# genomicepidemiology/ccphylo

Measured on AMD Instinct MI355X. Metric: taxa-pairs/sec (dist) + NJ iterations/sec at N taxa, 1/2/4/8 MI355X, higher is better.
Workload: dtype u2 packed codes -> MX-fp4 MFMA (exact integer counts), f64 LT and tree

## Files before the change

### ccphylo_amd/csrc/snp.hip

```cpp
#include <cstring>
#include <vector>
#include <type_traits>
#include "ccg_internal.h"
#include "ccg_shard_layout.h"

#define TILE 128
#define KC 16
#define KCP 8
#define RS 130
#define RSP 130

__device__ __forceinline__ uint32_t xor_or(uint32_t a, uint32_t b, uint32_t c) {
	return __builtin_amdgcn_bitop3_b32(a, b, c, 0xBE);
}

__device__ __forceinline__ uint32_t compress_even(uint64_t x) {
	x &= 0x5555555555555555ull;
	x = (x | (x >> 1)) & 0x3333333333333333ull;
	x = (x | (x >> 2)) & 0x0F0F0F0F0F0F0F0Full;
	x = (x | (x >> 4)) & 0x00FF00FF00FF00FFull;
	x = (x | (x >> 8)) & 0x0000FFFF0000FFFFull;
	x = (x | (x >> 16)) & 0x00000000FFFFFFFFull;
	return (uint32_t) x;
}
// ... 408 lines not shown
	int lo = 0, hi = npanels - 1;
	while(lo < hi) {
		const int mid = (lo + hi + 1) >> 1;
		if(pfx[mid] <= t) lo = mid; else hi = mid - 1;
	}
	const int I = lo, J = (int) (t - pfx[lo]);
	const Shard sh{rank, world};
	const auto arow = [&](int l) -> long long {
		const long long L = (long long) I * TILE + l, lb = L / SB, g = lb * world + rank, r = g * SB + (L - lb * SB);
		return r < n ? r : 0;
	};
	const uint2 *Bp = P + (size_t) J * TILE * Wp + wb;
	const int Wl = SPLIT ? (wb + Wk < Wp ? Wk : Wp - wb) : Wp;
	const int lane = threadIdx.x & 63, wid = threadIdx.x >> 6;
	const int wr = wid >> 1, wc = wid & 1;
	v16f_t acc[2][2];
#pragma unroll
	for(int a = 0; a < 2; ++a)
#pragma unroll
		for(int c = 0; c < 2; ++c)
#pragma unroll
			for(int r = 0; r < 16; ++r) acc[a][c][r] = 0.0f;
	uint4 va[4], vb[4];
	long long ar[4];
#pragma unroll
	for(int q = 0; q < 4; ++q) {
		const int e = q * 256 + threadIdx.x, row = e >> 3, wp = e & 7;
		ar[q] = arow(row);
		va[q] = *(const uint4 *) (P + (size_t) ar[q] * Wp + wb + 2 * wp);
		vb[q] = *(const uint4 *) (Bp + (size_t) row * Wp + 2 * wp);
	}
#pragma unroll
	for(int q = 0; q < 4; ++q) {
		const int e = q * 256 + threadIdx.x, row = e >> 3, wp = e & 7;
		As[0][(2 * wp) * RS + row] = make_uint2(va[q].x, va[q].y);
		As[0][(2 * wp + 1) * RS + row] = make_uint2(va[q].z, va[q].w);
		Bs[0][(2 * wp) * RS + row] = make_uint2(vb[q].x, vb[q].y);
		Bs[0][(2 * wp + 1) * RS + row] = make_uint2(vb[q].z, vb[q].w);
	}
	__syncthreads();
	const int h = lane >> 5, l32 = lane & 31;
	const int ra0 = 64 * wr + l32, rb0 = 64 * wc + l32;
	int buf = 0;
	for(int w0 = 0; w0 < Wl; w0 += KC, buf ^= 1) {
		const bool more = w0 + KC < Wl;
		if(more) {
#pragma unroll
			for(int q = 0; q < 4; ++q) {
				const int e = q * 256 + threadIdx.x, row = e >> 3, wp = e & 7;
				va[q] = *(const uint4 *) (P + (size_t) ar[q] * Wp + wb + w0 + KC + 2 * wp);
				vb[q] = *(const uint4 *) (Bp + (size_t) row * Wp + w0 + KC + 2 * wp);
			}
		}
		const uint2 *Ac = As[buf], *Bc = Bs[buf];
#pragma unroll 2
		for(int s = 0; s < KC / 2; ++s) {
			const int w = 2 * s + h;
			uint2 a[2], b[2];
#pragma unroll
			for(int tt = 0; tt < 2; ++tt) {
				a[tt] = Ac[w * RS + ra0 + 32 * tt];
				b[tt] = Bc[w * RS + rb0 + 32 * tt];
			}
#pragma unroll
			for(int comp = 0; comp < 3; ++comp) {
				v8i_t fa[2], fb[2];
#pragma unroll
				for(int tt = 0; tt < 2; ++tt) {
					fa[tt] = fp4_spread(comp == 0 ? a[tt].x : comp == 1 ? a[tt].y : a[tt].x ^ a[tt].y);
					fb[tt] = fp4_spread(comp == 0 ? b[tt].x : comp == 1 ? b[tt].y : b[tt].x ^ b[tt].y);
				}
#pragma unroll
				for(int ta = 0; ta < 2; ++ta)
#pragma unroll
					for(int tb = 0; tb < 2; ++tb)
						acc[ta][tb] = __builtin_amdgcn_mfma_scale_f32_32x32x64_f8f6f4(
						    fa[ta], fb[tb], acc[ta][tb], MFMA_FP4, MFMA_FP4, 0, MFMA_SCALE1, 0, MFMA_SCALE1);
			}
		}
		if(more) {
			uint2 *An = As[buf ^ 1], *Bn = Bs[buf ^ 1];
#pragma unroll
			for(int q = 0; q < 4; ++q) {
				const int e = q * 256 + threadIdx.x, row = e >> 3, wp = e & 7;
				An[(2 * wp) * RS + row] = make_uint2(va[q].x, va[q].y);
				An[(2 * wp + 1) * RS + row] = make_uint2(va[q].z, va[q].w);
				Bn[(2 * wp) * RS + row] = make_uint2(vb[q].x, vb[q].y);
				Bn[(2 * wp + 1) * RS + row] = make_uint2(vb[q].z, vb[q].w);
			}
		}
		__syncthreads();
	}
	const int L3 = 3 * 32 * Wl;
#pragma unroll
	for(int ta = 0; ta < 2; ++ta) {
#pragma unroll
		for(int r = 0; r < 16; ++r) {
			const int l = 64 * wr + 32 * ta + (r & 3) + 8 * (r >> 2) + 4 * h;
			const long long L = (long long) I * TILE + l, lb = L / SB, i = (lb * world + rank) * SB + (L - lb * SB);
			if(i >= n) continue;
			const long long base = sh.off(i);
#pragma unroll
			for(int tb = 0; tb < 2; ++tb) {
				const long long j = (long long) J * TILE + 64 * wc + 32 * tb + l32;
				if(j < i) {
					const unsigned d = (unsigned) ((L3 - (int) acc[ta][tb][r]) >> 2);
					if(SPLIT) atomicAdd(&cnt[base + j], d);
					else Dloc[base + j] = Elem<ET>::put(nFactor * (double) d, 0.5, bs);
				}
			}
		}
	}
}

#define TILE2 256
#define KC2 8
#define KC2L 16
#define RS2 260

__device__ __forceinline__ void tile_ij_super(long long t, long long Ihi, int &I, int &J) {
	int r, c;
	tile_ij(t, r, c);
	const long long P = r >> 2, I0 = 4 * P;
	if(I0 + 3 > Ihi) {
		I = r;
		J = c;
		return;
	}
	const long long u = t - I0 * (I0 + 1) / 2, F = P >> 1;
	if(u < 32 * F) {
		const int v = (int) (u & 31);
		I = (int) I0 + (v >> 3);
		J = 8 * (int) (u >> 5) + (v & 7);
		return;
	}
	long long w = u - 32 * F;
	int i = (int) I0;
	while(w >= i - 8 * F + 1) {
		w -= i - 8 * F + 1;
		++i;
	}
	I = i;
	J = (int) (8 * F + w);
}

__device__ __forceinline__ v8i_t fp4_xor_spread(const v8i_t &a, const v8i_t &b) {
	v8i_t v;
#pragma unroll
	for(int q = 0; q < 4; ++q) v[q] = (int) xor_or((uint32_t) a[q], (uint32_t) b[q], 0x22222222u);
	v[4] = v[5] = v[6] = v[7] = 0;
	return v;
}

template <int ET, bool SPLIT, bool BAND, int KCW = KC2>
__global__ __launch_bounds__(256, 1) void k_snp_mfma2(const uint2 *__restrict__ P, int Wp, int n, long long t0,
                                                      long long items, int S, int Wk, double nFactor, double bs,
                                                      typename Elem<ET>::T *__restrict__ D, long long rowBegin,
                                                      long long rowEnd, unsigned *__restrict__ cnt, long long cbase,
                                                      const long long *__restrict__ pfx, int npanels, int rank,
                                                      int world, int sorder) {
	constexpr int QS2 = TILE2 * KCW / 2 / 256, WPR = KCW / 2;
	__shared__ __attribute__((aligned(16))) uint2 As[2][KCW * RS2];
	__shared__ __attribute__((aligned(16))) uint2 Bs[2][KCW * RS2];
	const long long item = t0 + xcd_tile(blockIdx.x, items), t = SPLIT ? item / S : item;
	int I, J;
	if(BAND) {
		int lo = 0, hi = npanels - 1;
		while(lo < hi) {
			const int mid = (lo + hi + 1) >> 1;
			if(pfx[mid] <= t) lo = mid; else hi = mid - 1;
		}
		I = lo;
		J = (int) (t - pfx[lo]);
	} else if(sorder) {
		tile_ij_super(t, (rowEnd - 1) / TILE2, I, J);
	} else {
		tile_ij(t, I, J);
	}
	const int wb = SPLIT ? (int) (item % S) * Wk : 0;
	const int Wl = SPLIT ? (wb + Wk < Wp ? Wk : Wp - wb) : Wp;
	const Shard sh{rank, world};
	const auto arow = [&](int l) -> long long {
		const long long L = (long long) I * TILE2 + l;
		if(!BAND) return L;
		const long long lb = L / SB, r = (lb * world + rank) * SB + (L - lb * SB);
		return r < n ? r : 0;
	};
	const uint2 *Bp = P + (size_t) J * TILE2 * Wp + wb;
	long long ar[QS2];
	uint4 va[QS2], vb[QS2];
#pragma unroll
	for(int q = 0; q < QS2; ++q) {
		const int e = q * 256 + threadIdx.x, row = e / WPR, wp = e % WPR;
		ar[q] = arow(row);
		va[q] = *(const uint4 *) (P + (size_t) ar[q] * Wp + wb + 2 * wp);
		vb[q] = *(const uint4 *) (Bp + (size_t) row * Wp + 2 * wp);
	}
#pragma unroll
	for(int q = 0; q < QS2; ++q) {
		const int e = q * 256 + threadIdx.x, row = e / WPR, wp = e % WPR;
		As[0][(2 * wp) * RS2 + row] = make_uint2(va[q].x, va[q].y);
		As[0][(2 * wp + 1) * RS2 + row] = make_uint2(va[q].z, va[q].w);
		Bs[0][(2 * wp) * RS2 + row] = make_uint2(vb[q].x, vb[q].y);
		Bs[0][(2 * wp + 1) * RS2 + row] = make_uint2(vb[q].z, vb[q].w);
	}
	__syncthreads();
	const int lane = threadIdx.x & 63, wid = threadIdx.x >> 6;
	const int wr = wid >> 1, wc = wid & 1;
	const int h = lane >> 5, l32 = lane & 31;
	const int ra0 = 128 * wr + l32, rb0 = 128 * wc + l32;
	v16f_t acc[4][4];
#pragma unroll
	for(int a = 0; a < 4; ++a)
#pragma unroll
		for(int c = 0; c < 4; ++c)
#pragma unroll
			for(int r = 0; r < 16; ++r) acc[a][c][r] = 0.0f;
	int buf = 0;
	for(int w0 = 0; w0 < Wl; w0 += KCW, buf ^= 1) {
		const bool more = w0 + KCW < Wl;
		if(more) {
#pragma unroll
			for(int q = 0; q < QS2; ++q) {
				const int e = q * 256 + threadIdx.x, row = e / WPR, wp = e % WPR;
				va[q] = *(const uint4 *) (P + (size_t) ar[q] * Wp + wb + w0 + KCW + 2 * wp);
				vb[q] = *(const uint4 *) (Bp + (size_t) row * Wp + w0 + KCW + 2 * wp);
			}
		}
		const uint2 *Ac = As[buf], *Bc = Bs[buf];
#pragma unroll
		for(int s = 0; s < KCW / 2; ++s) {
			const int w = 2 * s + h;
			uint2 a[4], b[4];
#pragma unroll
			for(int x = 0; x < 4; ++x) {
				a[x] = Ac[w * RS2 + ra0 + 32 * x];
				b[x] = Bc[w * RS2 + rb0 + 32 * x];
			}
			v8i_t f0[4], g0[4], f1[4], g1[4];
#pragma unroll
			for(int x = 0; x < 4; ++x) {
				f0[x] = fp4_spread(a[x].x);
				g0[x] = fp4_spread(b[x].x);
			}
#pragma unroll
			for(int ta = 0; ta < 4; ++ta)
#pragma unroll
				for(int tb = 0; tb < 4; ++tb)
					acc[ta][tb] = __builtin_amdgcn_mfma_scale_f32_32x32x64_f8f6f4(
					    f0[ta], g0[tb], acc[ta][tb], MFMA_FP4, MFMA_FP4, 0, MFMA_SCALE1, 0, MFMA_SCALE1);
#pragma unroll
			for(int x = 0; x < 4; ++x) {
				f1[x] = fp4_spread(a[x].y);
				g1[x] = fp4_spread(b[x].y);
			}
#pragma unroll
			for(int ta = 0; ta < 4; ++ta)
#pragma unroll
				for(int tb = 0; tb < 4; ++tb)
					acc[ta][tb] = __builtin_amdgcn_mfma_scale_f32_32x32x64_f8f6f4(
					    f1[ta], g1[tb], acc[ta][tb], MFMA_FP4, MFMA_FP4, 0, MFMA_SCALE1, 0, MFMA_SCALE1);
#pragma unroll
			for(int x = 0; x < 4; ++x) {
				f0[x] = fp4_xor_spread(f0[x], f1[x]);
				g0[x] = fp4_xor_spread(g0[x], g1[x]);
			}
#pragma unroll
			for(int ta = 0; ta < 4; ++ta)
#pragma unroll
				for(int tb = 0; tb < 4; ++tb)
					acc[ta][tb] = __builtin_amdgcn_mfma_scale_f32_32x32x64_f8f6f4(
					    f0[ta], g0[tb], acc[ta][tb], MFMA_FP4, MFMA_FP4, 0, MFMA_SCALE1, 0, MFMA_SCALE1);
		}
		if(more) {
			uint2 *An = As[buf ^ 1], *Bn = Bs[buf ^ 1];
#pragma unroll
			for(int q = 0; q < QS2; ++q) {
				const int e = q * 256 + threadIdx.x, row = e / WPR, wp = e % WPR;
				An[(2 * wp) * RS2 + row] = make_uint2(va[q].x, va[q].y);
				An[(2 * wp + 1) * RS2 + row] = make_uint2(va[q].z, va[q].w);
				Bn[(2 * wp) * RS2 + row] = make_uint2(vb[q].x, vb[q].y);
				Bn[(2 * wp + 1) * RS2 + row] = make_uint2(vb[q].z, vb[q].w);
			}
		}
		__syncthreads();
	}
	const int L3 = 3 * 32 * Wl;
#pragma unroll
	for(int ta = 0; ta < 4; ++ta) {
#pragma unroll
		for(int r = 0; r < 16; ++r) {
			const int l = 128 * wr + 32 * ta + (r & 3) + 8 * (r >> 2) + 4 * h;
			const long long L = (long long) I * TILE2 + l;
			long long i = L;
			if(BAND) {
				const long long lb = L / SB;
				i = (lb * world + rank) * SB + (L - lb * SB);
			}
			if(i >= n || (!BAND && (i < rowBegin || i >= rowEnd))) continue;
			const long long base = BAND ? sh.off(i) : tri(i);
#pragma unroll
			for(int tb = 0; tb < 4; ++tb) {
				const long long j = (long long) J * TILE2 + 128 * wc + 32 * tb + l32;
				if(j < i) {
					const unsigned d = (unsigned) ((L3 - (int) acc[ta][tb][r]) >> 2);
					if(SPLIT) {
						atomicAdd(&cnt[base + j - cbase], d);
					} else {
						const double v = nFactor * (double) d;
						D[base + j] = Elem<ET>::put(v, 0.5, bs);
					}
				}
			}
		}
	}
}

#define NST3 4
#define KC3 8
template <int ET, bool SPLIT, bool BAND>
__global__ __launch_bounds__(256, 1) void k_snp_mfma3(const uint2 *__restrict__ P, int Wp, int n, long long t0,
                                                      long long items, int S, int Wk, double nFactor, double bs,
                                                      typename Elem<ET>::T *__restrict__ D, long long rowBegin,
                                                      long long rowEnd, unsigned *__restrict__ cnt, long long cbase,
                                                      const long long *__restrict__ pfx, int npanels, int rank,
                                                      int world, int sorder) {
	constexpr int NSL = KC3 / 2;
	static_assert(NSL == 4, "one slice per wave");
	__shared__ __attribute__((aligned(16))) uint4 L[NST3 * 2 * NSL * TILE2];
	const long long item = t0 + xcd_tile(blockIdx.x, items), t = SPLIT ? item / S : item;
	int I, J;
	if(BAND) {
		int lo = 0, hi = npanels - 1;
		while(lo < hi) {
			const int mid = (lo + hi + 1) >> 1;
			if(pfx[mid] <= t) lo = mid; else hi = mid - 1;
		}
		I = lo;
		J = (int) (t - pfx[lo]);
	} else if(sorder) {
		tile_ij_super(t, (rowEnd - 1) / TILE2, I, J);
	} else {
		tile_ij(t, I, J);
	}
	const int wb = SPLIT ? (int) (item % S) * Wk : 0;
	const int Wl = SPLIT ? (wb + Wk < Wp ? Wk : Wp - wb) : Wp;
	const Shard sh{rank, world};
	const int lane = threadIdx.x & 63, wid = threadIdx.x >> 6;
	const uint2 *srcA[4], *srcB[4];
#pragma unroll
	for(int q = 0; q < 4; ++q) {
		const long long Lr = (long long) I * TILE2 + q * 64 + lane;
		long long r = Lr;
		if(BAND) {
			const long long lb = Lr / SB;
			r = (lb * world + rank) * SB + (Lr - lb * SB);
			r = r < n ? r : 0;
		}
		srcA[q] = P + (size_t) r * Wp + wb + 2 * wid;
		srcB[q] = P + ((size_t) J * TILE2 + q * 64 + lane) * Wp + wb + 2 * wid;
	}
	const int nch = Wl / KC3;
	const unsigned lbase = (unsigned) (uintptr_t) (__attribute__((address_space(3))) uint4 *) L;
	auto glds = [&](const uint2 *src, unsigned lds) {
		unsigned keep;
		asm volatile("s_mov_b32 %0, m0\n\ts_mov_b32 m0, %2\n\ts_nop 0\n\tglobal_load_lds_dwordx4 %1, off\n\ts_mov_b32 m0, %0"
		             : "=&s"(keep)
		             : "v"(src), "s"(lds)
		             : "memory");
	};
	auto issue = [&](int c) {
		const int st = c % NST3, w0 = c * KC3;
#pragma unroll
		for(int q = 0; q < 4; ++q) {
			glds(srcA[q] + w0, __builtin_amdgcn_readfirstlane(lbase + (unsigned) ((((st * 2 + 0) * NSL + wid) * TILE2 + q * 64) * 16)));
			glds(srcB[q] + w0, __builtin_amdgcn_readfirstlane(lbase + (unsigned) ((((st * 2 + 1) * NSL + wid) * TILE2 + q * 64) * 16)));
		}
	};
	const int wr = wid >> 1, wc = wid & 1;
	const int h = lane >> 5, l32 = lane & 31;
	const int ra0 = 128 * wr + l32, rb0 = 128 * wc + l32;
	v16f_t acc[4][4];
#pragma unroll
	for(int ta = 0; ta < 4; ++ta)
#pragma unroll
		for(int tb = 0; tb < 4; ++tb)
#pragma unroll
			for(int r = 0; r < 16; ++r) acc[ta][tb][r] = 0.0f;
	auto land = [&](int c) {
		const int ahead = nch - 1 - c < NST3 - 2 ? nch - 1 - c : NST3 - 2;
		if(ahead >= 2) asm volatile("s_waitcnt vmcnt(16)" ::: "memory");
		else if(ahead == 1) asm volatile("s_waitcnt vmcnt(8)" ::: "memory");
		else asm volatile("s_waitcnt vmcnt(0)" ::: "memory");
		asm volatile("" ::: "memory");
		__builtin_amdgcn_s_barrier();
		asm volatile("" ::: "memory");
	};
	auto rd = [&](int gs, uint2 (&a)[4], uint2 (&b)[4]) {
		const int st = (gs >> 2) % NST3, sl = gs & 3;
		const uint2 *Ac = (const uint2 *) &L[((st * 2 + 0) * NSL + sl) * TILE2];
		const uint2 *Bc = (const uint2 *) &L[((st * 2 + 1) * NSL + sl) * TILE2];
#pragma unroll
		for(int x = 0; x < 4; ++x) {
			a[x] = Ac[(ra0 + 32 * x) * 2 + h];
			b[x] = Bc[(rb0 + 32 * x) * 2 + h];
		}
	};
#define MF3(TA, TB, F, G)                                                                                         \
	acc[TA][TB] = __builtin_amdgcn_mfma_scale_f32_32x32x64_f8f6f4(F, G, acc[TA][TB], MFMA_FP4, MFMA_FP4, 0, MFMA_SCALE1, \
	                                                              0, MFMA_SCALE1)
	for(int c = 0; c < NST3 - 1 && c < nch; ++c) issue(c);
	land(0);
	if(NST3 - 1 < nch) issue(NST3 - 1);
	uint2 a[4], b[4];
	v8i_t f0[4], g0[4];
	rd(0, a, b);
#pragma unroll
	for(int x = 0; x < 4; ++x) {
		f0[x] = fp4_spread(a[x].x);
		g0[x] = fp4_spread(b[x].x);
	}
	auto step = [&](auto SI, int gs, bool more, bool open) {
		constexpr int G0 = 3 * decltype(SI)::value;
		v8i_t f1[4], g1[4], x0[4], y0[4];
#pragma unroll
		for(int k = 0; k < 16; ++k) {
			MF3(k >> 2, k & 3, f0[k >> 2], g0[k & 3]);
			if(k < 8) {
				if(k & 1) g1[k >> 1] = fp4_spread(b[k >> 1].y);
				else f1[k >> 1] = fp4_spread(a[k >> 1].y);
			}
		}
#pragma unroll
		for(int k = 0; k < 8; ++k) {
			__builtin_amdgcn_sched_group_barrier(0x008, 1, G0);
			__builtin_amdgcn_sched_group_barrier(0x002, 7, G0);
		}
		__builtin_amdgcn_sched_group_barrier(0x008, 8, G0);
		if(open) {
			const int cn = (gs + 1) >> 2;
			land(cn);
			if(cn + NST3 - 1 < nch) issue(cn + NST3 - 1);
		}
		uint2 an[4], bn[4];
		if(more) rd(gs + 1, an, bn);
#pragma unroll
		for(int k = 0; k < 16; ++k) {
			MF3(k >> 2, k & 3, f1[k >> 2], g1[k & 3]);
			if(k < 8) {
				if(k & 1) y0[k >> 1] = fp4_xor_spread(g0[k >> 1], g1[k >> 1]);
				else x0[k >> 1] = fp4_xor_spread(f0[k >> 1], f1[k >> 1]);
			}
		}
		if(more) __builtin_amdgcn_sched_group_barrier(0x100, 8, G0 + 1);
#pragma unroll
		for(int k = 0; k < 8; ++k) {
			__builtin_amdgcn_sched_group_barrier(0x008, 1, G0 + 1);
			__builtin_amdgcn_sched_group_barrier(0x002, 4, G0 + 1);
		}
		__builtin_amdgcn_sched_group_barrier(0x008, 8, G0 + 1);
#pragma unroll
		for(int k = 0; k < 16; ++k) {
			MF3(k >> 2, k & 3, x0[k >> 2], y0[k & 3]);
			if(more && k < 8) {
				if(k & 1) g0[k >> 1] = fp4_spread(bn[k >> 1].x);
				else f0[k >> 1] = fp4_spread(an[k >> 1].x);
			}
		}
		if(more) {
#pragma unroll
			for(int k = 0; k < 8; ++k) {
				__builtin_amdgcn_sched_group_barrier(0x008, 1, G0 + 2);
				__builtin_amdgcn_sched_group_barrier(0x002, 7, G0 + 2);
			}
			__builtin_amdgcn_sched_group_barrier(0x008, 8, G0 + 2);
#pragma unroll
			for(int x = 0; x < 4; ++x) {
				a[x] = an[x];
				b[x] = bn[x];
			}
		}
	};
	for(int c = 0; c + 1 < nch; ++c) {
		step(std::integral_constant<int, 0>(), 4 * c + 0, true, false);
		step(std::integral_constant<int, 1>(), 4 * c + 1, true, false);
		step(std::integral_constant<int, 2>(), 4 * c + 2, true, false);
		step(std::integral_constant<int, 3>(), 4 * c + 3, true, true);
	}
	{
		const int g = 4 * (nch - 1);
		step(std::integral_constant<int, 0>(), g + 0, true, false);
		step(std::integral_constant<int, 1>(), g + 1, true, false);
		step(std::integral_constant<int, 2>(), g + 2, true, false);
		step(std::integral_constant<int, 3>(), g + 3, false, false);
	}
#undef MF3
	const int L3 = 3 * 32 * Wl;
#pragma unroll
	for(int ta = 0; ta < 4; ++ta) {
#pragma unroll
		for(int r = 0; r < 16; ++r) {
			const int l = 128 * wr + 32 * ta + (r & 3) + 8 * (r >> 2) + 4 * h;
			const long long Lr = (long long) I * TILE2 + l;
			long long i = Lr;
			if(BAND) {
				const long long lb = Lr / SB;
				i = (lb * world + rank) * SB + (Lr - lb * SB);
			}
			if(i >= n || (!BAND && (i < rowBegin || i >= rowEnd))) continue;
			const long long base = BAND ? sh.off(i) : tri(i);
#pragma unroll
			for(int tb = 0; tb < 4; ++tb) {
				const long long j = (long long) J * TILE2 + 128 * wc + 32 * tb + l32;
				if(j < i) {
					const unsigned d = (unsigned) ((L3 - (int) acc[ta][tb][r]) >> 2);
					if(SPLIT) {
						atomicAdd(&cnt[base + j - cbase], d);
					} else {
						const double v = nFactor * (double) d;
						D[base + j] = Elem<ET>::put(v, 0.5, bs);
					}
				}
			}
		}
	}
}

template <int ET>
__global__ void k_snp_finish(const unsigned *__restrict__ cnt, long long cbase, long long f0, long long f1,
                             double nFactor, double bs, typename Elem<ET>::T *__restrict__ D) {
	for(long long f = f0 + (long long) blockIdx.x * blockDim.x + threadIdx.x; f < f1;
	    f += (long long) gridDim.x * blockDim.x) {
		D[f] = Elem<ET>::put(nFactor * (double) cnt[f - cbase], 0.5, bs);
	}
}

template <int ET>
__device__ __forceinline__ void pair_store(typename Elem<ET>::T *D, typename Elem<ET>::T *N, long long f, uint32_t dist,
                                           uint32_t inc, unsigned norm, unsigned minLength, double bs) {
	typedef typename Elem<ET>::T T;
	if(ET == 8) {
		double v;
		if(minLength <= inc) {
			v = norm ? (double) ((unsigned long long) dist * norm) / inc : (double) dist;
		} else {
			v = -1.0;
		}
		D[f] = (T) v;
		if(N) N[f] = (T) (double) inc;
	} else if(ET == 4) {
		float v;
		if(minLength <= inc) {
			if(norm) {
				v = (float) ((unsigned long long) dist * norm);
				v = v / (float) inc;
			} else {
				v = (float) dist;
			}
		} else {
			v = -1.0f;
		}
		D[f] = (T) v;
		if(N) N[f] = (T) (float) inc;
	} else {
		double v;
		if(minLength <= inc) {
			v = norm ? ((double) ((unsigned long long) dist * norm) * bs + 0.5) / inc : (double) dist * bs + 0.5;
		} else {
			v = -1.0 * bs + 0;
		}
		D[f] = (T) cvt_i32_x86(v);
		if(N) N[f] = (T) cvt_i32_x86(inc * bs + 0.5);
	}
}

template <int ET, bool SPLIT, bool BAND = false>
__global__ __launch_bounds__(256, 2) void k_snp_tile_pair(const uint4 *__restrict__ P, int Wp, int n, long long t0,
                                                          long long items, int S, int Wk, unsigned norm,
                                                          unsigned minLength, double bs,
                                                          typename Elem<ET>::T *__restrict__ D,
                                                          typename Elem<ET>::T *__restrict__ Nm, long long rowBegin,
                                                          long long rowEnd, unsigned *__restrict__ cd,
                                                          unsigned *__restrict__ cn, long long cbase,
                                                          const long long *__restrict__ pfx = nullptr, int npanels = 0,
                                                          int rank = 0, int world = 1) {
	__shared__ __attribute__((aligned(16))) uint4 As[2][KCP * RSP];
	__shared__ __attribute__((aligned(16))) uint4 Bs[2][KCP * RSP];
	int I, J;
	const long long item = t0 + xcd_tile(blockIdx.x, items);
	if(BAND) {
		const long long tile = item / S;
		int lo = 0, hi = npanels - 1;
		while(lo < hi) {
			const int mid = (lo + hi + 1) >> 1;
			if(pfx[mid] <= tile) lo = mid; else hi = mid - 1;
		}
		I = lo;
		J = (int) (tile - pfx[lo]);
	} else {
		tile_ij(item / S, I, J);
	}
	const auto arow = [&](int l) -> long long {
		const long long L = (long long) I * TILE + l;
		if(!BAND) return L;
		const long long lb = L / SB, r = (lb * world + rank) * SB + (L - lb * SB);
		return r < n ? r : 0;
	};
	const int wb = (int) (item % S) * Wk, we = wb + Wk < Wp ? wb + Wk : Wp;
	const int Wl = we - wb;
	const int tx = threadIdx.x & 15, ty = threadIdx.x >> 4;
	const uint4 *Aq[4];
#pragma unroll
	for(int q = 0; q < 4; ++q) Aq[q] = P + (size_t) arow((q * 256 + threadIdx.x) >> 3) * Wp + wb;
	const uint4 *Bp = P + (size_t) J * TILE * Wp + wb;
	uint32_t ad[8][8], an[8][8];
#pragma unroll
	for(int a = 0; a < 8; ++a)
#pragma unroll
		for(int c = 0; c < 8; ++c) {
			ad[a][c] = 0;
			an[a][c] = 0;
		}
	uint4 va[4], vb[4];
#pragma unroll
	for(int q = 0; q < 4; ++q) {
		const int e = q * 256 + threadIdx.x, row = e >> 3, wp = e & 7;
		va[q] = Aq[q][wp];
		vb[q] = Bp[(size_t) row * Wp + wp];
	}
#pragma unroll
	for(int q = 0; q < 4; ++q) {
		const int e = q * 256 + threadIdx.x, row = e >> 3, wp = e & 7;
		As[0][wp * RSP + row] = va[q];
		Bs[0][wp * RSP + row] = vb[q];
	}
	__syncthreads();
	int buf = 0;
	for(int w0 = 0; w0 < Wl; w0 += KCP, buf ^= 1) {
		const bool more = w0 + KCP < Wl;
		if(more) {
#pragma unroll
			for(int q = 0; q < 4; ++q) {
				const int e = q * 256 + threadIdx.x, row = e >> 3, wp = e & 7;
				va[q] = Aq[q][w0 + KCP + wp];
				vb[q] = Bp[(size_t) row * Wp + w0 + KCP + wp];
			}
		}
		const uint4 *Ac = As[buf], *Bc = Bs[buf];
#pragma unroll 1
// ... 489 lines not shown
			uint32_t m = 0, d = 0;
			if(w < W32) {
				const uint4 a = A[w], b = B[w];
				m = a.z & b.z;
				d = xor_or(a.x, b.x, a.y ^ b.y) & m;
			}
			cnt += __popc(m);
			dist += __popc(d);
			const int hiL = d ? 32 * w + 32 - (__ffs(d)) + 1 : -1;
			int incl = wave_scan_max_incl(hiL, lane);
			int prevL = __shfl_up(incl, 1, 64);
			if(lane == 0) prevL = -1;
			if(cL > prevL) prevL = cL;
			int qhi = 0;
			{
				int prev = prevL;
				for(uint32_t x = d; x;) {
					const int k = __clz(x);
					x &= ~(0x80000000u >> k);
					const int cur = 32 * w + k + 1;
					qhi = prev >= 0 && cur - prev <= proxi;
					prev = cur;
				}
			}
			const int packed = hiL >= 0 ? 2 * hiL + qhi : -1;
			const int incl2 = wave_scan_max_incl(packed, lane);
			int prevP = __shfl_up(incl2, 1, 64);
			if(lane == 0) prevP = -1;
			const int cP = cL >= 0 ? 2 * cL + cQ : -1;
			if(cP > prevP) prevP = cP;
			{
				int prev = prevL, qprev = prevP >= 0 ? (prevP & 1) : 0;
				for(uint32_t x = d; x;) {
					const int k = __clz(x);
					x &= ~(0x80000000u >> k);
					const int cur = 32 * w + k + 1;
					const int qc = prev >= 0 && cur - prev <= proxi;
					if(qc) {
						uint32_t rm, rd;
						range_counts(A, B, W32, prev, cur, rm, rd);
						cnt -= rm;
						dist -= rd;
						if(qprev) {
							range_counts(A, B, W32, prev, prev, rm, rd);
							cnt += rm;
							dist += rd;
						}
					}
					prev = cur;
					qprev = qc;
				}
			}
			const int top = __shfl(incl2, 63, 64);
			if(top >= 0 && (top >> 1) > cL) {
				cL = top >> 1;
				cQ = top & 1;
			}
		}
		if(lane == 0 && cL >= 0 && (long long) len + proxi - cL <= proxi) {
			uint32_t rm, rd;
			const long long e = (long long) len + proxi;
			range_counts(A, B, W32, cL, e < 32LL * W32 ? (int) e : 32 * W32 - 1, rm, rd);
			cnt -= rm;
			dist -= rd;
			if(cQ) {
				range_counts(A, B, W32, cL, cL, rm, rd);
				cnt += rm;
				dist += rd;
			}
		}
#pragma unroll
		for(int o = 32; o > 0; o >>= 1) {
			dist += __shfl_xor(dist, o, 64);
			cnt += __shfl_xor(cnt, o, 64);
		}
		if(lane == 0) pair_store<ET>(D, Nm, f, (uint32_t) dist, (uint32_t) cnt, norm, minLength, bs);
	}
}

static inline long long cdivll(long long a, long long b) { return (a + b - 1) / b; }

static int dist_kernel_choice() {
	const char *mf = getenv("CCG_DIST_MFMA");
	return mf ? atoi(mf) : 2;
}

template <int ET, bool PAIR = false>
static int snp_launch_mfma2(ccg_ctx *ctx, const ccg_snp_args *a, const void *planes, int Wp, double nFactor, void *D,
                            long long rb, long long re, int rank, int world, void *N = NULL) {
	typedef typename Elem<ET>::T T;
	const long long n = a->n;
	long long t_begin = 0, t_end = 0, f0 = 0, f1 = 0;
	int npanels = 0;
	long long *d_pfx = NULL;
	if(world > 0) {
		const long long nb = (n + SB - 1) / SB;
		long long nloc = 0;
		if(rank < nb) {
			const long long owned = (nb - 1 - rank) / world + 1, last = (owned - 1) * world + rank;
			nloc = (owned - 1) * SB + (n - last * SB < SB ? n - last * SB : SB);
		}
		npanels = (int) cdivll(nloc, TILE2);
		if(npanels == 0) return CCG_OK;
		std::vector<long long> pfx(npanels + 1, 0);
		for(long long I = 0; I < npanels; ++I) {
			const long long Lmax = (I + 1) * TILE2 - 1 < nloc - 1 ? (I + 1) * TILE2 - 1 : nloc - 1;
			const long long lb = Lmax / SB, rmax = (lb * world + rank) * SB + (Lmax - lb * SB);
			pfx[I + 1] = pfx[I] + cdivll(rmax, TILE2);
		}
		CCG_CHECK(hipMalloc(&d_pfx, (size_t) (npanels + 1) * sizeof(long long)));
		if(hipMemcpyAsync(d_pfx, pfx.data(), (size_t) (npanels + 1) * sizeof(long long), hipMemcpyHostToDevice,
		                  ctx->stream) != hipSuccess) {
			hipFree(d_pfx);
			return CCG_EHIP;
		}
		t_end = pfx[npanels];
		f1 = ccg_shard_elems(n, rank, world);
	} else {
		const long long Ilo = rb / TILE2, Ihi = (re - 1) / TILE2;
		t_begin = Ilo * (Ilo + 1) / 2;
		t_end = (Ihi + 1) * (Ihi + 2) / 2;
		f0 = tri(rb);
		f1 = tri(re);
	}
	if(PAIR) {
		t_begin *= 2;
		t_end *= 2;
	}
	const long long tiles = t_end - t_begin;
	hipDeviceProp_t prop;
	if(hipGetDeviceProperties(&prop, ctx->device) != hipSuccess) {
		hipFree(d_pfx);
		return CCG_EHIP;
	}
	const long long slots = prop.multiProcessorCount;
	const char *kce = getenv("CCG_DIST_KC"), *ore = getenv("CCG_DIST_ORDER");
	const int kc = !PAIR && kce && atoi(kce) == KC2L && Wp % KC2L == 0 ? KC2L : KC2;
	const char *gle = getenv("CCG_DIST_GLDS");
	const bool glds = !PAIR && !(gle && atoi(gle) == 0) && kc == KC3;
	const int sorder = !PAIR && world == 0 && ore && atoi(ore) == 1 && (rb / TILE2) % 4 == 0;
	const int chunks = Wp / kc;
	int S = 1;
	if(tiles < 16 * slots) {
		S = (int) cdivll(16 * slots, tiles);
		if(S > chunks / 4) S = chunks / 4;
		if(S < 1) S = 1;
	}
	int Wk = (int) cdivll(chunks, S) * kc;
	if(Wk > MFMA_KMAX) Wk = (MFMA_KMAX / kc) * kc;
	S = (int) cdivll(Wp, Wk);
	const long long batch = 1 << 16;
	unsigned *cnt = NULL;
	int rc = CCG_OK;
#define MF2_TRY(x) do { if((x) != hipSuccess) { rc = CCG_EHIP; goto out; } } while(0)
	if(S > 1) {
		const size_t cz = (size_t) (f1 - f0) * (PAIR ? 2 : 1) * sizeof(unsigned);
		if(hipMalloc(&cnt, cz) != hipSuccess) {
			cnt = NULL;
			rc = CCG_ENOMEM;
			goto out;
		}
		MF2_TRY(hipMemsetAsync(cnt, 0, cz, ctx->stream));
	}
	for(long long t = t_begin * S; t < t_end * S; t += batch) {
		const long long items = t_end * S - t < batch ? t_end * S - t : batch;
		const uint2 *pl = (const uint2 *) planes;
		if(PAIR) {
			typedef typename Elem<ET>::T T;
			const uint4 *pp = (const uint4 *) planes;
			unsigned *cn = cnt ? cnt + (f1 - f0) : NULL;
			T *Nn = world > 0 ? NULL : (T *) N;
			if(world > 0 && S > 1)
				k_snp_mfma2_pair<ET, true, true><<<(unsigned) items, 256, 0, ctx->stream>>>(
				    pp, Wp, (int) n, t, items, S, Wk, a->norm, a->minLength, a->byteScale, (T *) D, Nn, 0, n, cnt, cn, 0,
				    d_pfx, npanels, rank, world);
			else if(world > 0)
				k_snp_mfma2_pair<ET, false, true><<<(unsigned) items, 256, 0, ctx->stream>>>(
				    pp, Wp, (int) n, t, items, 1, Wp, a->norm, a->minLength, a->byteScale, (T *) D, Nn, 0, n, cnt, cn, 0,
				    d_pfx, npanels, rank, world);
			else if(S > 1)
				k_snp_mfma2_pair<ET, true, false><<<(unsigned) items, 256, 0, ctx->stream>>>(
				    pp, Wp, (int) n, t, items, S, Wk, a->norm, a->minLength, a->byteScale, (T *) D, Nn, rb, re, cnt, cn,
				    f0, NULL, 0, 0, 1);
			else
				k_snp_mfma2_pair<ET, false, false><<<(unsigned) items, 256, 0, ctx->stream>>>(
				    pp, Wp, (int) n, t, items, 1, Wp, a->norm, a->minLength, a->byteScale, (T *) D, Nn, rb, re, cnt, cn,
				    f0, NULL, 0, 0, 1);
			MF2_TRY(hipGetLastError());
			continue;
		}
#define MF2_LAUNCH(KCV)                                                                                              \
	if(world > 0) {                                                                                                  \
		if(S > 1)                                                                                                    \
			k_snp_mfma2<ET, true, true, KCV><<<(unsigned) items, 256, 0, ctx->stream>>>(                             \
			    pl, Wp, (int) n, t, items, S, Wk, nFactor, a->byteScale, (T *) D, 0, n, cnt, 0, d_pfx, npanels, rank,  \
			    world, 0);                                                                                           \
		else                                                                                                         \
			k_snp_mfma2<ET, false, true, KCV><<<(unsigned) items, 256, 0, ctx->stream>>>(                            \
			    pl, Wp, (int) n, t, items, 1, Wp, nFactor, a->byteScale, (T *) D, 0, n, cnt, 0, d_pfx, npanels, rank,  \
			    world, 0);                                                                                           \
	} else {                                                                                                         \
		if(S > 1)                                                                                                    \
			k_snp_mfma2<ET, true, false, KCV><<<(unsigned) items, 256, 0, ctx->stream>>>(                            \
			    pl, Wp, (int) n, t, items, S, Wk, nFactor, a->byteScale, (T *) D, rb, re, cnt, f0, NULL, 0, 0, 1,       \
			    sorder);                                                                                             \
		else                                                                                                         \
			k_snp_mfma2<ET, false, false, KCV><<<(unsigned) items, 256, 0, ctx->stream>>>(                           \
			    pl, Wp, (int) n, t, items, 1, Wp, nFactor, a->byteScale, (T *) D, rb, re, cnt, f0, NULL, 0, 0, 1,       \
			    sorder);                                                                                             \
	}
		if(glds) {
			if(world > 0) {
				if(S > 1)
					k_snp_mfma3<ET, true, true><<<(unsigned) items, 256, 0, ctx->stream>>>(
					    pl, Wp, (int) n, t, items, S, Wk, nFactor, a->byteScale, (T *) D, 0, n, cnt, 0, d_pfx, npanels,
					    rank, world, 0);
				else
					k_snp_mfma3<ET, false, true><<<(unsigned) items, 256, 0, ctx->stream>>>(
					    pl, Wp, (int) n, t, items, 1, Wp, nFactor, a->byteScale, (T *) D, 0, n, cnt, 0, d_pfx, npanels,
					    rank, world, 0);
			} else {
				if(S > 1)
					k_snp_mfma3<ET, true, false><<<(unsigned) items, 256, 0, ctx->stream>>>(
					    pl, Wp, (int) n, t, items, S, Wk, nFactor, a->byteScale, (T *) D, rb, re, cnt, f0, NULL, 0, 0, 1,
					    sorder);
				else
					k_snp_mfma3<ET, false, false><<<(unsigned) items, 256, 0, ctx->stream>>>(
					    pl, Wp, (int) n, t, items, 1, Wp, nFactor, a->byteScale, (T *) D, rb, re, cnt, f0, NULL, 0, 0, 1,
					    sorder);
			}
		} else if(kc == KC2L) {
			MF2_LAUNCH(KC2L)
		} else {
			MF2_LAUNCH(KC2)
		}
#undef MF2_LAUNCH
		MF2_TRY(hipGetLastError());
	}
	if(S > 1) {
		const long long g = cdivll(f1 - f0, 256);
		if(PAIR)
			k_snp_pair_finish<ET><<<(unsigned) (g < 65536 ? g : 65536), 256, 0, ctx->stream>>>(
			    cnt, cnt + (f1 - f0), f0, f1, a->norm, a->minLength, a->byteScale, (T *) D,
			    world > 0 ? (T *) NULL : (T *) N);
		else
			k_snp_finish<ET><<<(unsigned) (g < 65536 ? g : 65536), 256, 0, ctx->stream>>>(cnt, f0, f0, f1, nFactor,
			                                                                                a->byteScale, (T *) D);
		MF2_TRY(hipGetLastError());
	}
	MF2_TRY(hipStreamSynchronize(ctx->stream));
out:
#undef MF2_TRY
	if(rc != CCG_OK) hipStreamSynchronize(ctx->stream);
	if(cnt && hipFree(cnt) != hipSuccess && rc == CCG_OK) rc = CCG_EHIP;
	if(d_pfx && hipFree(d_pfx) != hipSuccess && rc == CCG_OK) rc = CCG_EHIP;
	return rc;
}

template <int ET>
static int snp_launch(ccg_ctx *ctx, const ccg_snp_args *a, const void *planes, int Wp, double nFactor, void *D, void *N,
                      long long rb, long long re) {
	typedef typename Elem<ET>::T T;
	long long Ilo = rb / TILE, Ihi = (re - 1) / TILE;
	long long t_begin = Ilo * (Ilo + 1) / 2, t_end = (Ihi + 1) * (Ihi + 2) / 2;
	const long long batch = 1 << 14;
	if(a->pair && a->proxi) {
		const long long f0 = tri(rb), f1 = tri(re), g = cdivll(f1 - f0, 4);
		const int W32 = (a->len + 31) / 32;
		if(f1 > f0) {
			k_snp_pair_proxi<ET><<<(unsigned) (g < 16384 ? g : 16384), 256, 0, ctx->stream>>>(
			    (const uint4 *) planes, Wp, W32, a->len, (int) a->proxi, f0, f1, a->norm, a->minLength, a->byteScale,
			    (T *) D, (T *) N);
			CCG_CHECK(hipGetLastError());
		}
		return CCG_OK;
	}
	hipDeviceProp_t prop;
	CCG_CHECK(hipGetDeviceProperties(&prop, ctx->device));
	const long long slots = 2LL * prop.multiProcessorCount;
	const long long tiles = t_end - t_begin;
	const int kc = a->pair ? KCP : KC;
	const int chunks = Wp / kc;
	int S = 1;
	if(tiles < 16 * slots) {
		S = (int) cdivll(16 * slots, tiles);
		if(S > chunks / 4) S = chunks / 4;
		if(S < 1) S = 1;
	}
	const int Wk = (int) cdivll(chunks, S) * kc;
	S = (int) cdivll(Wp, Wk);
	const long long f0 = tri(rb), f1 = tri(re);
	const long long i_begin = t_begin * S, i_end = t_end * S;
	if(a->pair && dist_kernel_choice() == 2)
		return snp_launch_mfma2<ET, true>(ctx, a, planes, Wp, nFactor, D, rb, re, 0, 0, N);
	if(a->pair) {
		unsigned *cd = NULL, *cn = NULL;
		if(S > 1) {
			CCG_CHECK(hipMalloc(&cd, (size_t) (f1 - f0) * 2 * sizeof(unsigned)));
			cn = cd + (f1 - f0);
			CCG_CHECK(hipMemsetAsync(cd, 0, (size_t) (f1 - f0) * 2 * sizeof(unsigned), ctx->stream));
		}
		const char *mfp = getenv("CCG_DIST_MFMA");
		const bool pmfma = (mfp ? atoi(mfp) : 1) && Wk < MFMA_KMAX;
		for(long long t = i_begin; t < i_end; t += batch) {
			long long items = i_end - t < batch ? i_end - t : batch;
			if(pmfma) {
				if(S > 1)
					k_snp_mfma_pair<ET, true><<<(unsigned) items, 256, 0, ctx->stream>>>(
					    (const uint4 *) planes, Wp, a->n, t, items, S, Wk, a->norm, a->minLength, a->byteScale, (T *) D,
					    (T *) N, rb, re, cd, cn, f0);
				else
					k_snp_mfma_pair<ET, false><<<(unsigned) items, 256, 0, ctx->stream>>>(
					    (const uint4 *) planes, Wp, a->n, t, items, 1, Wp, a->norm, a->minLength, a->byteScale, (T *) D,
					    (T *) N, rb, re, cd, cn, f0);
			} else if(S > 1) {
				k_snp_tile_pair<ET, true><<<(unsigned) items, 256, 0, ctx->stream>>>(
				    (const uint4 *) planes, Wp, a->n, t, items, S, Wk, a->norm, a->minLength, a->byteScale, (T *) D,
				    (T *) N, rb, re, cd, cn, f0);
			} else {
				k_snp_tile_pair<ET, false><<<(unsigned) items, 256, 0, ctx->stream>>>(
				    (const uint4 *) planes, Wp, a->n, t, items, 1, Wp, a->norm, a->minLength, a->byteScale, (T *) D,
				    (T *) N, rb, re, cd, cn, f0);
			}
			CCG_CHECK(hipGetLastError());
		}
		if(S > 1) {
			long long g = cdivll(f1 - f0, 256);
			k_snp_pair_finish<ET><<<(unsigned) (g < 65536 ? g : 65536), 256, 0, ctx->stream>>>(
			    cd, cn, f0, f1, a->norm, a->minLength, a->byteScale, (T *) D, (T *) N);
			CCG_CHECK(hipGetLastError());
			CCG_CHECK(hipStreamSynchronize(ctx->stream));
			CCG_CHECK(hipFree(cd));
		}
		return CCG_OK;
	}
	if(dist_kernel_choice() == 2) return snp_launch_mfma2<ET>(ctx, a, planes, Wp, nFactor, D, rb, re, 0, 0);
	const int use_mfma = dist_kernel_choice();
	int Sm = S, Wkm = Wk;
	if(use_mfma && Wkm > MFMA_KMAX) {
		Wkm = (MFMA_KMAX / kc) * kc;
		Sm = (int) cdivll(Wp, Wkm);
	}
	if(use_mfma) {
		S = Sm;
	}
	const long long mi_begin = t_begin * S, mi_end = t_end * S;
	unsigned *cnt = NULL;
	if(S > 1) {
		CCG_CHECK(hipMalloc(&cnt, (size_t) (f1 - f0) * sizeof(unsigned)));
		CCG_CHECK(hipMemsetAsync(cnt, 0, (size_t) (f1 - f0) * sizeof(unsigned), ctx->stream));
	}
	for(long long t = use_mfma ? mi_begin : i_begin; t < (use_mfma ? mi_end : i_end); t += batch) {
		const long long iend = use_mfma ? mi_end : i_end;
		long long items = iend - t < batch ? iend - t : batch;
		if(use_mfma) {
			if(S > 1)
				k_snp_mfma<ET, true><<<(unsigned) items, 256, 0, ctx->stream>>>((const uint2 *) planes, Wp, a->n, t, items,
				                                                             S, Wkm, nFactor, a->byteScale, (T *) D, rb,
				                                                             re, cnt, f0);
			else
				k_snp_mfma<ET, false><<<(unsigned) items, 256, 0, ctx->stream>>>((const uint2 *) planes, Wp, a->n, t,
				                                                              items, 1, Wp, nFactor, a->byteScale,
				                                                              (T *) D, rb, re, cnt, f0);
		} else if(S > 1) {
			k_snp_tile<ET, true><<<(unsigned) items, 256, 0, ctx->stream>>>((const uint2 *) planes, Wp, a->n, t, items, S,
			                                                             Wk, nFactor, a->byteScale, (T *) D, rb, re,
			                                                             cnt, f0);
		} else {
			k_snp_tile<ET, false><<<(unsigned) items, 256, 0, ctx->stream>>>((const uint2 *) planes, Wp, a->n, t, items,
			                                                              1, Wp, nFactor, a->byteScale, (T *) D, rb,
			                                                              re, cnt, f0);
		}
		CCG_CHECK(hipGetLastError());
	}
	if(S > 1) {
		long long g = cdivll(f1 - f0, 256);
		k_snp_finish<ET><<<(unsigned) (g < 65536 ? g : 65536), 256, 0, ctx->stream>>>(cnt, f0, f0, f1, nFactor,
		                                                                                a->byteScale, (T *) D);
		CCG_CHECK(hipGetLastError());
		CCG_CHECK(hipStreamSynchronize(ctx->stream));
		CCG_CHECK(hipFree(cnt));
	}
	return CCG_OK;
}

template <int ET>
static int snp_launch_band(ccg_ctx *ctx, const ccg_snp_args *a, const void *planes, int Wp, double nFactor, void *D,
                           int rank, int world) {
	typedef typename Elem<ET>::T T;
	const long long n = a->n;
	auto row_of = [&](long long L) {
		const long long lb = L / SB;
		return (lb * world + rank) * SB + (L - lb * SB);
	};
	long long nloc = 0;
	const long long nb = (n + SB - 1) / SB;
	if(rank < nb) {
		const long long owned = (nb - 1 - rank) / world + 1, last = (owned - 1) * world + rank;
		nloc = (owned - 1) * SB + (n - last * SB < SB ? n - last * SB : SB);
	}
	if(a->pair && a->proxi) {
		const int W32 = (a->len + 31) / 32;
		const Shard sh{rank, world};
		for(long long g = rank; g < nb;) {
			long long g2 = g;
			while(world == 1 && g2 + 1 < nb) ++g2;
// ... 402 lines not shown
```

Before: 185.6 million.

## Interleave LDS loads and global-to-LDS issues with MFMAs in mfma3 pipeline

Restructures the k_snp_mfma3 inner step so that fp4 spreading, LDS reads for the next slice, and global_load_lds issues for the next stage are split into halves and interleaved one-per-MFMA with explicit sched barriers. The previous sched_group_barrier scheme is replaced. In steady state, the wait-and-barrier happens before the second MFMA group and the prefetch issues are spread across it, instead of being done in bulk. The change also adds optional s_memtime stamp instrumentation behind a compile flag. The main risk is that the strict sched_barrier ordering constrains the compiler and lengthens register live ranges.

```diff
diff --git a/ccphylo_amd/csrc/snp.hip b/ccphylo_amd/csrc/snp.hip
--- a/ccphylo_amd/csrc/snp.hip
+++ b/ccphylo_amd/csrc/snp.hip
@@ -584,6 +584,23 @@
 	return v;
 }
 
+__device__ __forceinline__ void fp4_spread_half(v8i_t &v, uint32_t x, int hf) {
+	if(hf == 0) {
+		v[0] = (int) and_or(x << 3, 0x88888888u, 0x22222222u);
+		v[1] = (int) and_or(x << 2, 0x88888888u, 0x22222222u);
+		v[4] = v[5] = v[6] = v[7] = 0;
+	} else {
+		v[2] = (int) and_or(x << 1, 0x88888888u, 0x22222222u);
+		v[3] = (int) and_or(x, 0x88888888u, 0x22222222u);
+	}
+}
+
+__device__ __forceinline__ void fp4_xor_spread_half(v8i_t &v, const v8i_t &a, const v8i_t &b, int hf) {
+	if(hf == 0) v[4] = v[5] = v[6] = v[7] = 0;
+#pragma unroll
+	for(int q = 2 * hf; q < 2 * hf + 2; ++q) v[q] = (int) xor_or((uint32_t) a[q], (uint32_t) b[q], 0x22222222u);
+}
+
 template <int ET, bool SPLIT, bool BAND, int KCW = KC2>
 __global__ __launch_bounds__(256, 1) void k_snp_mfma2(const uint2 *__restrict__ P, int Wp, int n, long long t0,
                                                       long long items, int S, int Wk, double nFactor, double bs,
@@ -750,6 +767,22 @@
 
 #define NST3 4
 #define KC3 8
+#ifdef CCG_DIST_STAMPS
+#define ST3_SLOTS 8
+__device__ unsigned long long *ccg_dist_stamp_buf;
+__device__ long long ccg_dist_stamp_item0;
+#define ST3(K)                                                                              \
+	do {                                                                                    \
+		unsigned long long tn_;                                                             \
+		__builtin_amdgcn_sched_barrier(0);                                                  \
+		asm volatile("s_memtime %0\n\ts_waitcnt lgkmcnt(0)" : "=s"(tn_)::"memory");         \
+		__builtin_amdgcn_sched_barrier(0);                                                  \
+		if((K) >= 0) stamp_sum[(K) < 0 ? 0 : (K)] += tn_ - stamp_prev;                      \
+		stamp_prev = tn_;                                                                   \
+	} while(0)
+#else
+#define ST3(K)
+#endif
 template <int ET, bool SPLIT, bool BAND>
 __global__ __launch_bounds__(256, 1) void k_snp_mfma3(const uint2 *__restrict__ P, int Wp, int n, long long t0,
                                                       long long items, int S, int Wk, double nFactor, double bs,
@@ -801,13 +834,14 @@
 		             : "v"(src), "s"(lds)
 		             : "memory");
 	};
+	const unsigned lwave = (unsigned) __builtin_amdgcn_readfirstlane((int) (lbase + (unsigned) (wid * TILE2 * 16)));
+	auto issue1 = [&](int c, int i) {
+		const int st = c % NST3, w0 = c * KC3, q = i >> 1, p = i & 1;
+		glds((p ? srcB[q] : srcA[q]) + w0, lwave + (unsigned) ((((st * 2 + p) * NSL) * TILE2 + q * 64) * 16));
+	};
 	auto issue = [&](int c) {
-		const int st = c % NST3, w0 = c * KC3;
-#pragma unroll
-		for(int q = 0; q < 4; ++q) {
-			glds(srcA[q] + w0, __builtin_amdgcn_readfirstlane(lbase + (unsigned) ((((st * 2 + 0) * NSL + wid) * TILE2 + q * 64) * 16)));
-			glds(srcB[q] + w0, __builtin_amdgcn_readfirstlane(lbase + (unsigned) ((((st * 2 + 1) * NSL + wid) * TILE2 + q * 64) * 16)));
-		}
+#pragma unroll
+		for(int i = 0; i < 8; ++i) issue1(c, i);
 	};
 	const int wr = wid >> 1, wc = wid & 1;
 	const int h = lane >> 5, l32 = lane & 31;
@@ -828,15 +862,15 @@
 		__builtin_amdgcn_s_barrier();
 		asm volatile("" ::: "memory");
 	};
+	auto rd1 = [&](int gs, int p, uint2 (&v)[4]) {
+		const int st = (gs >> 2) % NST3, sl = gs & 3;
+		const uint2 *Pc = (const uint2 *) &L[((st * 2 + p) * NSL + sl) * TILE2];
+#pragma unroll
+		for(int x = 0; x < 4; ++x) v[x] = Pc[((p ? rb0 : ra0) + 32 * x) * 2 + h];
+	};
 	auto rd = [&](int gs, uint2 (&a)[4], uint2 (&b)[4]) {
-		const int st = (gs >> 2) % NST3, sl = gs & 3;
-		const uint2 *Ac = (const uint2 *) &L[((st * 2 + 0) * NSL + sl) * TILE2];
-		const uint2 *Bc = (const uint2 *) &L[((st * 2 + 1) * NSL + sl) * TILE2];
-#pragma unroll
-		for(int x = 0; x < 4; ++x) {
-			a[x] = Ac[(ra0 + 32 * x) * 2 + h];
-			b[x] = Bc[(rb0 + 32 * x) * 2 + h];
-		}
+		rd1(gs, 0, a);
+		rd1(gs, 1, b);
 	};
 #define MF3(TA, TB, F, G)                                                                                         \
 	acc[TA][TB] = __builtin_amdgcn_mfma_scale_f32_32x32x64_f8f6f4(F, G, acc[TA][TB], MFMA_FP4, MFMA_FP4, 0, MFMA_SCALE1, \
@@ -852,60 +886,61 @@
 		f0[x] = fp4_spread(a[x].x);
 		g0[x] = fp4_spread(b[x].x);
 	}
-	auto step = [&](auto SI, int gs, bool more, bool open) {
-		constexpr int G0 = 3 * decltype(SI)::value;
+#ifdef CCG_DIST_STAMPS
+	unsigned long long stamp_sum[ST3_SLOTS] = {0, 0, 0, 0, 0, 0, 0, 0}, stamp_prev = 0;
+#endif
+#define GAP3() __builtin_amdgcn_sched_barrier(0)
+	auto step = [&](auto OPEN, auto MORE, int gs) {
+		constexpr int open = decltype(OPEN)::value;
+		constexpr bool more = decltype(MORE)::value;
 		v8i_t f1[4], g1[4], x0[4], y0[4];
 #pragma unroll
 		for(int k = 0; k < 16; ++k) {
 			MF3(k >> 2, k & 3, f0[k >> 2], g0[k & 3]);
-			if(k < 8) {
-				if(k & 1) g1[k >> 1] = fp4_spread(b[k >> 1].y);
-				else f1[k >> 1] = fp4_spread(a[k >> 1].y);
-			}
-		}
-#pragma unroll
-		for(int k = 0; k < 8; ++k) {
-			__builtin_amdgcn_sched_group_barrier(0x008, 1, G0);
-			__builtin_amdgcn_sched_group_barrier(0x002, 7, G0);
-		}
-		__builtin_amdgcn_sched_group_barrier(0x008, 8, G0);
+			const int j = k >> 1;
+			if(j == 0 || j > 4) fp4_spread_half(f1[j ? j - 4 : 0], a[j ? j - 4 : 0].y, k & 1);
+			else fp4_spread_half(g1[j - 1], b[j - 1].y, k & 1);
+			GAP3();
+		}
+		const int cn = (gs + 1) >> 2;
 		if(open) {
-			const int cn = (gs + 1) >> 2;
-			land(cn);
-			if(cn + NST3 - 1 < nch) issue(cn + NST3 - 1);
+			ST3(3);
+			GAP3();
+			if(open == 2) {
+				asm volatile("s_waitcnt vmcnt(16)" ::: "memory");
+				asm volatile("" ::: "memory");
+				__builtin_amdgcn_s_barrier();
+				asm volatile("" ::: "memory");
+			} else {
+				land(cn);
+			}
+			GAP3();
+			ST3(4);
 		}
 		uint2 an[4], bn[4];
-		if(more) rd(gs + 1, an, bn);
 #pragma unroll
 		for(int k = 0; k < 16; ++k) {
 			MF3(k >> 2, k & 3, f1[k >> 2], g1[k & 3]);
-			if(k < 8) {
-				if(k & 1) y0[k >> 1] = fp4_xor_spread(g0[k >> 1], g1[k >> 1]);
-				else x0[k >> 1] = fp4_xor_spread(f0[k >> 1], f1[k >> 1]);
-			}
-		}
-		if(more) __builtin_amdgcn_sched_group_barrier(0x100, 8, G0 + 1);
-#pragma unroll
-		for(int k = 0; k < 8; ++k) {
-			__builtin_amdgcn_sched_group_barrier(0x008, 1, G0 + 1);
-			__builtin_amdgcn_sched_group_barrier(0x002, 4, G0 + 1);
-		}
-		__builtin_amdgcn_sched_group_barrier(0x008, 8, G0 + 1);
+			const int j = k >> 1;
+			if(j == 0 || j > 4) fp4_xor_spread_half(x0[j ? j - 4 : 0], f0[j ? j - 4 : 0], f1[j ? j - 4 : 0], k & 1);
+			else fp4_xor_spread_half(y0[j - 1], g0[j - 1], g1[j - 1], k & 1);
+			if(more && k == 0) rd1(gs + 1, 0, an);
+			if(more && k == 1) rd1(gs + 1, 1, bn);
+			if(open == 2 && (k & 1)) issue1(cn + NST3 - 1, k >> 1);
+			GAP3();
+		}
+		if(open == 2) ST3(5);
 #pragma unroll
 		for(int k = 0; k < 16; ++k) {
 			MF3(k >> 2, k & 3, x0[k >> 2], y0[k & 3]);
-			if(more && k < 8) {
-				if(k & 1) g0[k >> 1] = fp4_spread(bn[k >> 1].x);
-				else f0[k >> 1] = fp4_spread(an[k >> 1].x);
-			}
+			if(more) {
+				const int j = k >> 1;
+				if(j == 0 || j > 4) fp4_spread_half(f0[j ? j - 4 : 0], an[j ? j - 4 : 0].x, k & 1);
+				else fp4_spread_half(g0[j - 1], bn[j - 1].x, k & 1);
+			}
+			GAP3();
 		}
 		if(more) {
-#pragma unroll
-			for(int k = 0; k < 8; ++k) {
-				__builtin_amdgcn_sched_group_barrier(0x008, 1, G0 + 2);
-				__builtin_amdgcn_sched_group_barrier(0x002, 7, G0 + 2);
-			}
-			__builtin_amdgcn_sched_group_barrier(0x008, 8, G0 + 2);
 #pragma unroll
 			for(int x = 0; x < 4; ++x) {
 				a[x] = an[x];
@@ -913,20 +948,45 @@
 			}
 		}
 	};
-	for(int c = 0; c + 1 < nch; ++c) {
-		step(std::integral_constant<int, 0>(), 4 * c + 0, true, false);
-		step(std::integral_constant<int, 1>(), 4 * c + 1, true, false);
-		step(std::integral_constant<int, 2>(), 4 * c + 2, true, false);
-		step(std::integral_constant<int, 3>(), 4 * c + 3, true, true);
-	}
+	typedef std::integral_constant<int, 0> O0;
+	typedef std::integral_constant<int, 1> O1;
+	typedef std::integral_constant<int, 2> O2;
+	typedef std::true_type MT;
+	ST3(-1);
+	int c = 0;
+	for(; c + NST3 < nch; ++c) {
+		step(O0(), MT(), 4 * c + 0);
+		ST3(0);
+		step(O0(), MT(), 4 * c + 1);
+		ST3(1);
+		step(O0(), MT(), 4 * c + 2);
+		ST3(2);
+		step(O2(), MT(), 4 * c + 3);
+		ST3(6);
+	}
+	for(; c + 1 < nch; ++c) {
+		step(O0(), MT(), 4 * c + 0);
+		step(O0(), MT(), 4 * c + 1);
+		step(O0(), MT(), 4 * c + 2);
+		step(O1(), MT(), 4 * c + 3);
+	}
+#ifdef CCG_DIST_STAMPS
+	if(ccg_dist_stamp_buf && lane == 0 && (wid == 0 || wid == 3)) {
+		stamp_sum[7] = nch > NST3 ? nch - NST3 : 0;
+		unsigned long long *sb =
+		    ccg_dist_stamp_buf + ((t0 - ccg_dist_stamp_item0 + blockIdx.x) * 2 + (wid ? 1 : 0)) * ST3_SLOTS;
+		for(int k = 0; k < ST3_SLOTS; ++k) sb[k] = stamp_sum[k];
+	}
+#endif
 	{
 		const int g = 4 * (nch - 1);
-		step(std::integral_constant<int, 0>(), g + 0, true, false);
-		step(std::integral_constant<int, 1>(), g + 1, true, false);
-		step(std::integral_constant<int, 2>(), g + 2, true, false);
-		step(std::integral_constant<int, 3>(), g + 3, false, false);
+		step(O0(), MT(), g + 0);
+		step(O0(), MT(), g + 1);
+		step(O0(), MT(), g + 2);
+		step(O0(), std::false_type(), g + 3);
 	}
 #undef MF3
+#undef GAP3
 	const int L3 = 3 * 32 * Wl;
 #pragma unroll
 	for(int ta = 0; ta < 4; ++ta) {
@@ -1722,7 +1782,21 @@
 	const long long batch = 1 << 16;
 	unsigned *cnt = NULL;
 	int rc = CCG_OK;
+#ifdef CCG_DIST_STAMPS
+	unsigned long long *d_st = NULL;
+	const char *sto = getenv("CCG_DIST_STAMPS_OUT");
+	const size_t stn = (size_t) (t_end - t_begin) * S * 2 * ST3_SLOTS;
+	const long long st_item0 = t_begin * S;
+#endif
 #define MF2_TRY(x) do { if((x) != hipSuccess) { rc = CCG_EHIP; goto out; } } while(0)
+#ifdef CCG_DIST_STAMPS
+	if(glds && sto) {
+		MF2_TRY(hipMalloc(&d_st, stn * sizeof(unsigned long long)));
+		MF2_TRY(hipMemsetAsync(d_st, 0, stn * sizeof(unsigned long long), ctx->stream));
+	}
+	MF2_TRY(hipMemcpyToSymbol(HIP_SYMBOL(ccg_dist_stamp_buf), &d_st, sizeof(d_st)));
+	MF2_TRY(hipMemcpyToSymbol(HIP_SYMBOL(ccg_dist_stamp_item0), &st_item0, sizeof(st_item0)));
+#endif
 	if(S > 1) {
 		const size_t cz = (size_t) (f1 - f0) * (PAIR ? 2 : 1) * sizeof(unsigned);
 		if(hipMalloc(&cnt, cz) != hipSuccess) {
@@ -1819,9 +1893,23 @@
 		MF2_TRY(hipGetLastError());
 	}
 	MF2_TRY(hipStreamSynchronize(ctx->stream));
+#ifdef CCG_DIST_STAMPS
+	if(d_st) {
+		std::vector<unsigned long long> hs(stn);
+		MF2_TRY(hipMemcpy(hs.data(), d_st, stn * sizeof(unsigned long long), hipMemcpyDeviceToHost));
+		FILE *sf = fopen(sto, "ab");
+		if(sf) {
+			fwrite(hs.data(), sizeof(unsigned long long), stn, sf);
+			fclose(sf);
+		}
+	}
+#endif
 out:
 #undef MF2_TRY
 	if(rc != CCG_OK) hipStreamSynchronize(ctx->stream);
+#ifdef CCG_DIST_STAMPS
+	if(d_st) hipFree(d_st);
+#endif
 	if(cnt && hipFree(cnt) != hipSuccess && rc == CCG_OK) rc = CCG_EHIP;
 	if(d_pfx && hipFree(d_pfx) != hipSuccess && rc == CCG_OK) rc = CCG_EHIP;
 	return rc;
```

After: 201.9 million (median of 6 runs). 1.09x the previous value.
